# puzzlepaint/surfelmeshing

Hardware: AMD Instinct MI355X
Metric: RGB-D frames/s integrated @640x480, 5M live surfels; achieved HBM GB/s (higher is better)
Workload: dtype f32; 1 GPU; C2: synthetic room stream 640x480, raw depth + colour frames resident in HBM, full preprocessing + Integrate per frame, 4912850 live surfels (6250000 slots), steady-state re-traversal; max_surfel_count=6250000, streams=1, parallelism=1 independent stream per GPU

## Files before the change

### surfelmeshing_amd/csrc/smx_recon.hip

```cpp
#include <math.h>
#include <cmath>
#include <stdlib.h>
#include <string.h>

#include <algorithm>
#include <atomic>
#include <vector>

#include "smx_recon_state.hpp"
#include "smx_mesh.hpp"
#include <hip/hip_ext.h>

using namespace smx;

namespace {

struct FrameCtx {
  Mat34 L;
  Mat34 G;
  float fx, fy, cx, cy;
  Unproj up;
  float inv_depth_scaling;
  float sensor_noise_factor;
  float cos_normal_compat;
// ... 654 lines not shown
  SMX_STAMP(stamps, 2);
  if (lane == 0) {
    tb.count[tile * kCountStride] = 0;
    if (tile == 0) { *next_ovf_count = 0; seg_work_count[0] = 0; seg_work_count[1] = 0; }
    if (c.stats) {
      atomicAdd(&st->n_pairs, n_total);
      atomicMax(&st->max_tile_pairs, n_total);
      if (tile == 0) st->n_overflow_pairs = n_ovf;
    }
  }
#pragma unroll
  for (int q = 0; q < kPairCache; ++q) if (have[q]) assoc_stage(t, c, rec[q]);
  for_uncached_pairs(S, c, tb, tile, n_binned, overflowed, n_ovf, [&](const PairRec& r) { assoc_stage(t, c, r); });
  __syncthreads();
  SMX_STAMP(stamps, 3);
  uint32_t cand[kPairCache];
  float4 cp4[kPairCache], cn4[kPairCache];
#pragma unroll
  for (int q = 0; q < kPairCache; ++q) cand[q] = have[q] ? merge_candidate(t, c, rec[q]) : kInvalid;
#pragma unroll
  for (int q = 0; q < kPairCache; ++q) {
    const uint32_t g = cand[q] == kInvalid ? 0u : cand[q];
    cp4[q] = *S.group(kGroupP, g); cn4[q] = *S.group(kGroupN, g);
  }
#pragma unroll
  for (int q = 0; q < kPairCache; ++q) { keep(cp4[q]); keep(cn4[q]); }
#pragma unroll
  for (int q = 0; q < kPairCache; ++q) if (cand[q] != kInvalid) merge_decide(rec[q], cp4[q], cn4[q], merge_flag);
  for_uncached_pairs(S, c, tb, tile, n_binned, overflowed, n_ovf, [&](const PairRec& r) { merge_stage(t, S, c, r, merge_flag); });
  __syncthreads();
  SMX_STAMP(stamps, 4);
  if (in_image) {
    const size_t k = (size_t)y * c.W + x;
    sc.first_depth[k] = __int_as_float(t.zmin[lane]);
    sc.supporting[k] = t.sup[lane];
    sc.counts[k] = t.cnt[lane];
    sc.depth_sums[k] = (long long)t.sum[lane];
    sc.confl_key[k] = t.confl[lane];
  }
  SMX_STAMP(stamps, 5);
  ts_end(c.ts, kTsTilesEnd, blockIdx.x, gridDim.x);
}

__device__ __forceinline__ float depth_sum_avg(const Scratch& sc, size_t k) {
  return q_to_float(sc.depth_sums[k]) / (float)sc.counts[k];
}

__global__ void __launch_bounds__(kBlock)
k_blend_start(float ds, Img<uint16_t> depth, Scratch sc, BlendBufs b, int W, int H, unsigned long long* ts) {
  ts_end(ts, kTsBlendEnd, blockIdx.y * gridDim.x + blockIdx.x, gridDim.x * gridDim.y);
  const int x = blockIdx.x * 64 + (threadIdx.x & 63);
  const int y = blockIdx.y * 4 + (threadIdx.x >> 6);
  if (!(x >= 1 && y >= 1 && x < W - 1 && y < H - 1)) return;
  const size_t k = (size_t)y * W + x;
  const uint16_t own = depth(y, x);
  if (own == 0 || sc.supporting[k] == kInvalid) return;
  bool measurement_border = false, surfel_border = false;
  for (int wy = y - 1; wy <= y + 1; ++wy)
    for (int wx = x - 1; wx <= x + 1; ++wx) {
      if (depth(wy, wx) == 0) measurement_border = true;
      else if (sc.supporting[(size_t)wy * W + wx] == kInvalid) surfel_border = true;
    }
  if (surfel_border) {
    b.new_distance_map[k] = 1;
    const float avg = depth_sum_avg(sc, k);
    b.new_deltas[k] = avg - (float)own / ds;
  }
  if (measurement_border) {
    b.distance_map[k] = 1;
    const float avg = depth_sum_avg(sc, k);
    b.deltas[k] = avg - (float)own / ds;
// ... 264 lines not shown
#endif
    }
#ifdef SMX_STAMPS
    if (dbg) { dbg[0] = t_in; dbg[1] = wall_clock64(); dbg[2] = polls; }
#endif
  }
}

constexpr int kScanPxPerThread = 4;
constexpr int kScanPxPerBlock = kBlock * kScanPxPerThread;

struct NewFlagsArgs {
  Img<const uint16_t> depth; Img<uint16_t> depth_out; int copy_back;
  uint8_t* flags; uint32_t* local_rank; uint32_t* block_sums;
  unsigned long long* dbg;
};
__device__ __forceinline__ void new_flags_scan_body(const NewFlagsArgs& a, const Scratch& sc, int W, int H, DevState* st, uint32_t block) {
  const Img<const uint16_t>& depth = a.depth;
  const Img<uint16_t>& depth_out = a.depth_out;
  const int copy_back = a.copy_back;
  uint8_t* __restrict__ flags = a.flags;
  uint32_t* __restrict__ local_rank = a.local_rank;
  uint32_t* __restrict__ block_sums = a.block_sums;
  __shared__ uint32_t wave_tot[kBlock / 64];
  const int P = W * H;
  const int k0 = (block * kBlock + threadIdx.x) * kScanPxPerThread;
  uint32_t f[kScanPxPerThread];
  uint32_t mine = 0;
  uint32_t dv[kScanPxPerThread], sv[kScanPxPerThread], cv[kScanPxPerThread];
#pragma unroll
  for (int j = 0; j < kScanPxPerThread; ++j) {
    const int k = min(k0 + j, P - 1);
    const int y = k / W, x = k - y * W;
    dv[j] = depth(y, x); sv[j] = sc.supporting[k]; cv[j] = sc.confl_key[k];
  }
#pragma unroll
  for (int j = 0; j < kScanPxPerThread; ++j) { keep(dv[j]); keep(sv[j]); keep(cv[j]); }
#pragma unroll
  for (int j = 0; j < kScanPxPerThread; ++j) {
    const int k = k0 + j;
    bool fl = false;
    if (k < P) {
      const int y = k / W, x = k - y * W;
      const uint16_t d = (uint16_t)dv[j];
      if (copy_back) depth_out(y, x) = d;
      fl = x >= 1 && y >= 1 && x < W - 1 && y < H - 1 && d > 0 && sv[j] == kInvalid && cv[j] == kInvalid;
      flags[k] = fl ? 1 : 0;
    }
    f[j] = fl ? 1u : 0u;
    mine += f[j];
  }
  const uint32_t lane = threadIdx.x & 63, wave = threadIdx.x >> 6;
  uint32_t incl = mine;
#pragma unroll
  for (int off = 1; off < 64; off <<= 1) {
    const uint32_t t = __shfl_up(incl, off);
    if (lane >= (uint32_t)off) incl += t;
  }
  if (lane == 63) wave_tot[wave] = incl;
  __syncthreads();
  uint32_t wave_off = 0, total = 0;
#pragma unroll
  for (int w = 0; w < kBlock / 64; ++w) {
    if ((uint32_t)w < wave) wave_off += wave_tot[w];
    total += wave_tot[w];
  }
  uint32_t run = wave_off + incl - mine;
#pragma unroll
  for (int j = 0; j < kScanPxPerThread; ++j) {
    const int k = k0 + j;
    if (k < P) local_rank[k] = run;
    run += f[j];
  }
  if (threadIdx.x == 0) {
    block_sums[block] = total;
    if (block == 0) st->create_base_next = st->surfel_count;
  }
}

struct FrameIn {
  Img<const uint16_t> depth; Img<const float2> normals; Img<const float> radius; Img<const uchar3> color;
};

struct PixelIn {
  uint16_t depth; float first; uint32_t key; uint32_t count; float2 nxy; uchar3 col; float radius;
};
__device__ __forceinline__ PixelIn load_pixel(const FrameCtx& c, const Scratch& sc, const FrameIn& in, int x, int y) {
  const size_t k = (size_t)y * c.W + x;
  PixelIn p;
  p.depth = in.depth(y, x); p.first = sc.first_depth[k]; p.key = sc.confl_key[k]; p.count = sc.counts[k];
  p.nxy = in.normals(y, x); p.col = in.color(y, x); p.radius = in.radius(y, x);
  return p;
}

__device__ __forceinline__ void keep(const PixelIn& p) {
  keep((uint32_t)p.depth); keep(p.first); keep(p.key); keep(p.count); keep(p.nxy); keep(p.radius);
  keep((uint32_t)p.col.x | ((uint32_t)p.col.y << 8) | ((uint32_t)p.col.z << 16));
}

struct SurfelRegs {
  float4 P;
  float4 N;
  float4 C;
  bool dirty;
  bool replaced;
  Vec3 new_smooth;
};

__device__ __forceinline__ void integrate_or_conflict(SurfelRegs& R, const FrameCtx& c, const PixelIn& px,
                                                      bool integrate, int x, int y,
                                                      const Vec3& cam, uint32_t i, DevState* st) {
  if (!integrate) return;
  const float measurement_depth = c.inv_depth_scaling * (float)px.depth;
  if (measurement_depth <= 0) return;
  bool conflicting = false;
  const float first = px.first;
  if (first < (1 - c.sensor_noise_factor) * measurement_depth) {
    if (first == cam.z) {
      const uint32_t key = px.key;
      if (key != kInvalid && (key & 0x7FFFFFFFu) == i) conflicting = true;
    }
    integrate = false;
  }
// ... 104 lines not shown
    const float4 p4 = R.P, n4 = R.N;
    if (!is_active(__float_as_uint(p4.w), c.frame, c.window)) continue;
    Proj p;
    const Vec3 g = {p4.x, p4.y, p4.z};
    if (!project_pos(g, c, p)) continue;
    if (n4.w < 0) continue;
    int ox = p.px, oy = p.py;
    const bool second = quadrant(p, c, ox, oy);
    const PixelIn px0 = load_pixel(c, sc, in, p.px, p.py);
    const PixelIn px1 = load_pixel(c, sc, in, ox, oy);
    integrate_or_conflict(R, c, px0, true, p.px, p.py, p.l, i, st);
    integrate_or_conflict(R, c, px1, second, ox, oy, p.l, i, st);
    if (R.dirty) {
      L.hot_epoch[i >> L.hot_shift] = (uint8_t)L.epoch;
      if (L.dirty8) L.dirty8[i] = 1;
      out_store16(S.group(kGroupP, i), R.P); out_store16(S.group(kGroupN, i), R.N);
      out_store16(S.group(kGroupC, i), R.C);
      if (R.replaced) {
        *S.group(kGroupS, i) = make_float4(R.new_smooth.x, R.new_smooth.y, R.new_smooth.z, 0.0f);
        S.set_neighbors(i, make_uint4(kInvalid, kInvalid, kInvalid, kInvalid));
      }
    }
    L.flags8[i] = make_flags(__float_as_uint(R.P.w), __float_as_uint(R.C.z), c.frame, c.reg_window);
  }
#pragma unroll
  for (int off = 32; off > 0; off >>= 1) merged_here += __shfl_xor(merged_here, off);
  if ((threadIdx.x & 63) == 0 && merged_here) {
    atomicAdd(&st->merge_count, merged_here);
    if (c.stats) atomicAdd(&st->n_merged, merged_here);
  }
  ts_end(c.ts, kTsIntEnd, block, min(n_blocks, n_steps));
}

template <bool kUseList>
__device__ __forceinline__ void update_neighbors_body(const Surfels& S, const FrameCtx& c, const Scratch& sc, const FrameIn& in,
                                                      const Lists& L, const DevState* st, uint32_t block, uint32_t n_blocks) {
  const int kDX[4] = {-1, 1, 0, 0}, kDY[4] = {0, 0, -1, 1};
  const uint32_t n_scan = kUseList ? 0u : st->create_base_next;
  if (block == 0 && threadIdx.x < kSubLists) { L.rec_chunks.count[threadIdx.x * kCountStride] = 0; L.acc_chunks.count[threadIdx.x * kCountStride] = 0; }
  uint32_t ent, cntv;
  const uint32_t n_steps = vis_begin<kUseList>(L, n_scan, block, ent, cntv);
  for (uint32_t w = block; w < n_steps; w += n_blocks) {
    const uint32_t cur = ent;
    ent = (w + n_blocks < n_steps) ? vis_load<kUseList>(L, w + n_blocks) : 0u;
    uint32_t i;
    if (!vis_entry<kUseList>(cur, w, cntv, n_scan, threadIdx.x, i)) continue;
    const float4 p4 = *S.group(kGroupP, i), n4 = *S.group(kGroupN, i);
    const uint4 t4 = *reinterpret_cast<const uint4*>(S.group(kGroupT, i));
    if (!is_active(__float_as_uint(p4.w), c.frame, c.window)) continue;
    const Vec3 g = {p4.x, p4.y, p4.z};
    const Vec3 cam = mul(c.L, g);
    if (!(cam.z > 0)) continue;
    const float u = c.fx * (cam.x / cam.z) + c.cx, v = c.fy * (cam.y / cam.z) + c.cy;
    if (!(u >= 1.0f && v >= 1.0f && u < (float)(c.W - 1) && v < (float)(c.H - 1))) continue;
    const int x = (int)u, y = (int)v;
    const float measurement_depth = c.inv_depth_scaling * (float)in.depth(y, x);
    const float obs_r2 = in.radius(y, x);
    uint32_t cand[4];
#pragma unroll
    for (int d = 0; d < 4; ++d) cand[d] = sc.supporting[(size_t)(y + kDY[d]) * c.W + (x + kDX[d])];
    const float occlusion_depth = (1 + c.sensor_noise_factor) * measurement_depth;
    if (cam.z > occlusion_depth) continue;
    const float surfel_distance = sqrtf(cam.x * cam.x + cam.y * cam.y + cam.z * cam.z);
    const Vec3 gn = {n4.x, n4.y, n4.z};
    const Vec3 ln = rotate(c.L, gn);
    const float dot_angle = (1.0f / surfel_distance) * (cam.x * ln.x + cam.y * ln.y + cam.z * ln.z);
    if (dot_angle > 0) continue;
    const float r2 = n4.w;
    if (r2 < 0) continue;
    if (obs_r2 / r2 > 1.5f * 1.5f) continue;

    uint32_t ni[4] = {t4.x, t4.y, t4.z, t4.w};
    float4 np4[4], cp4[4], cn4[4];
#pragma unroll
    for (int q = 0; q < 4; ++q) np4[q] = *S.group(kGroupP, ni[q] == kInvalid ? i : ni[q]);
#pragma unroll
    for (int d = 0; d < 4; ++d) {
      const uint32_t gidx = (cand[d] == kInvalid) ? i : cand[d];
      cp4[d] = *S.group(kGroupP, gidx);
      cn4[d] = *S.group(kGroupN, gidx);
    }
    float nd2[4];
#pragma unroll
    for (int q = 0; q < 4; ++q) {
      if (ni[q] == kInvalid) nd2[q] = __builtin_inff();
      else {
        const float dx = g.x - np4[q].x, dy = g.y - np4[q].y, dz = g.z - np4[q].z;
        nd2[q] = dx * dx + dy * dy + dz * dz;
      }
    }
#pragma unroll
    for (int d = 0; d < 4; ++d) {
      const uint32_t nb = cand[d];
      if (nb == kInvalid || nb == i) continue;
      const float dx = cp4[d].x - g.x, dy = cp4[d].y - g.y, dz = cp4[d].z - g.z;
      const float d2 = dx * dx + dy * dy + dz * dz;
      if (d2 > c.rf2 * r2) continue;
      const float nd = gn.x * cn4[d].x + gn.y * cn4[d].y + gn.z * cn4[d].z;
      if (nd <= 0) continue;
      int best_n = -1; float best_d2 = -1;
#pragma unroll
      for (int q = 0; q < 4; ++q) {
        if (best_n == -2) continue;
        if (nb == ni[q]) { best_n = -2; }
        else if (nd2[q] > best_d2) { best_n = q; best_d2 = nd2[q]; }
      }
      if (best_n >= 0 && d2 < best_d2) {
#pragma unroll
        for (int q = 0; q < 4; ++q) if (q == best_n) { ni[q] = nb; nd2[q] = d2; }
      }
    }
    if (ni[0] != t4.x || ni[1] != t4.y || ni[2] != t4.z || ni[3] != t4.w) {
      S.set_neighbors(i, make_uint4(ni[0], ni[1], ni[2], ni[3]));
      L.hot_epoch[i >> L.hot_shift] = (uint8_t)L.epoch;
    }
  }
  ts_end(c.ts, kTsUpdEnd, block, min(n_blocks, n_steps));
}

struct CreateArgs {
  const uint8_t* flags; const uint32_t* ranks; const uint32_t* block_sums; uint32_t* block_offsets_out;
  int n_scan_blocks; uint32_t max_surfels; uint8_t* flags8; uint8_t* dirty8;
  uint32_t* next_vis_chunk_count;
  int n_pixels;
  uint8_t* hot_epoch; uint32_t epoch; int hot_shift;
};
__device__ __forceinline__ void new_create_body(const Surfels& S, const FrameCtx& c, const Scratch& sc, const FrameIn& in,
                                                const CreateArgs& a, DevState* st, uint32_t block, uint32_t n_blocks) {
  const uint8_t* __restrict__ flags = a.flags;
  const uint32_t* __restrict__ ranks = a.ranks;
  const uint32_t* __restrict__ block_sums = a.block_sums;
  uint32_t* __restrict__ block_offsets_out = a.block_offsets_out;
  const int n_scan_blocks = a.n_scan_blocks;
  const uint32_t max_surfels = a.max_surfels;
  uint8_t* __restrict__ flags8 = a.flags8;
  extern __shared__ uint32_t block_offsets[];
  __shared__ uint32_t wave_tot[kBlock / 64];
  static_assert(kScanPxPerBlock % kBlock == 0, "a creating workgroup's pixels lie inside one scan block");
  if (block != 0 && n_blocks * (uint32_t)kBlock >= (uint32_t)(c.W * c.H) &&
      block_sums[(block * (uint32_t)kBlock) / (uint32_t)kScanPxPerBlock] == 0) return;
  const int per = (n_scan_blocks + kBlock - 1) / kBlock;
  const uint32_t base = st->create_base_next;
  uint32_t mine = 0, total;
  if (per <= 8) {
    uint32_t v[8];
#pragma unroll
    for (int j = 0; j < 8; ++j) {
      const int bidx = threadIdx.x * per + j;
// ... 765 lines not shown
    __syncthreads();
    if (threadIdx.x == 0) carry += total;
    __syncthreads();
  }
  if (threadIdx.x == 0) *total_out = carry;
}
__global__ void __launch_bounds__(kBlock)
k_delta_gather(Surfels S, uint8_t* __restrict__ dirty8, const uint32_t* __restrict__ seg_offset, float* __restrict__ out,
               uint32_t total, const DevState* st) {
  __shared__ uint32_t wave_tot[kBlock / 64];
  const uint32_t N = st->surfel_count, i0 = blockIdx.x * kSeg + threadIdx.x * 4;
  uint32_t bits = 0;
  if (i0 < N) {
    const uchar4 d = *reinterpret_cast<const uchar4*>(&dirty8[i0]);
    bits = (d.x != 0 ? 1u : 0u) | ((i0 + 1 < N && d.y != 0) ? 2u : 0u) | ((i0 + 2 < N && d.z != 0) ? 4u : 0u) |
           ((i0 + 3 < N && d.w != 0) ? 8u : 0u);
    if (bits) *reinterpret_cast<uchar4*>(&dirty8[i0]) = make_uchar4(0, 0, 0, 0);
  }
  uint32_t seg_total;
  uint32_t off = seg_offset[blockIdx.x] + block_excl_scan((uint32_t)__popc(bits), wave_tot, seg_total);
  const int want[8] = {kSmoothX, kSmoothY, kSmoothZ, kRadiusSq, kNormalX, kNormalY, kNormalZ, kLastUpdateStamp};
#pragma unroll
  for (int j = 0; j < 4; ++j)
    if (bits & (1u << j)) {
      const uint32_t i = i0 + j;
      out[off] = __uint_as_float(i);
#pragma unroll
      for (int k = 0; k < 8; ++k) out[(size_t)(k + 1) * total + off] = S.f(want[k], i);
      ++off;
    }
}

__global__ void __launch_bounds__(kBlock)
k_decode_conflicting(const uint32_t* __restrict__ key, uint32_t* __restrict__ out, int P) {
  const int k = blockIdx.x * kBlock + threadIdx.x;
  if (k < P) out[k] = (key[k] == kInvalid) ? kInvalid : (key[k] & 0x7FFFFFFFu);
}

__global__ void __launch_bounds__(kBlock)
k_global_ranks(const uint32_t* __restrict__ local_rank, const uint32_t* __restrict__ block_offsets,
               uint32_t* __restrict__ out, int P) {
  const int k = blockIdx.x * kBlock + threadIdx.x;
  if (k < P) out[k] = block_offsets[k / kScanPxPerBlock] + local_rank[k];
}

}

enum : int {
  kSlotScanVisible = 0, kSlotAssocTiles, kSlotBlend, kSlotIntegrate,
  kSlotUpdateNeighbors, kSlotNeighborScan,
  kSlotRegAccumulate, kSlotRegStep,
  kSlotRegUpdate,
  kSlotCull,
  kSlotEmpty,
  kSlotCount
};
static const char* const kSlotNames[kSlotCount] = {
  "scan_visible", "assoc_tiles", "blend", "integrate+new_flags", "update_neighbors+create",
  "neighbor_scan", "reg_accumulate", "reg_step", "reg_update", "cull_segments", "empty_slot"};

struct SlotTimer {
  smx_recon r; hipStream_t st; int slot; bool kev, prof, by_launch;
  SlotTimer(smx_recon r_, hipStream_t st_, int slot_, bool launch_carries = false) : r(r_), st(st_), slot(slot_) {
    kev = (r->timing_enabled & 2) != 0;
    prof = (r->prof_slot == slot) && r->prof_ev && r->prof_n < r->prof_cap;
    by_launch = prof && launch_carries;
    if (kev) (void)hipEventRecord(r->kev[2 * slot], st);
    if (prof && !by_launch) (void)hipEventRecord(r->prof_ev[2 * r->prof_n], st);
  }
// ... 145 lines not shown
  SMX_TRY(r->mem.alloc(&r->fb.count, ((size_t)r->nsegB + 1) * kCountStride, true));
  r->L.vis_region = (uint32_t)(div_up(r->nseg, kSubLists) * kSeg);
  SMX_TRY(r->mem.alloc(&r->L.vis_list, (size_t)kSubLists * r->L.vis_region, true));
  SMX_TRY(r->mem.alloc(&r->L.recent_list, (size_t)r->nsegB * kSegB, false));
  SMX_TRY(r->mem.alloc(&r->L.vis_seg, (size_t)r->nseg, true));
  SMX_TRY(r->mem.alloc(&r->L.seg_box, (size_t)r->nseg * 8, true));
  SMX_TRY(r->mem.alloc(&r->L.seg_act, (size_t)r->nseg, true));
  SMX_TRY(r->mem.alloc(&r->L.seg_streak, (size_t)r->nseg, true));
  SMX_TRY(r->mem.alloc(&r->sw.surv_list, (size_t)r->nseg + 65536, true));
  SMX_TRY(r->mem.alloc(&r->sw.copy_list, (size_t)r->nseg + 65536, true));
  SMX_TRY(r->mem.alloc(&r->sw.count, 2, true));
  SMX_TRY(r->mem.alloc_host(&r->dir_host, 2, true));
  r->dir_host[0] = 0;
  r->dir_host[1] = 0;
  SMX_TRY(hip_rc(hipHostGetDevicePointer(reinterpret_cast<void**>(&r->dir_dev), r->dir_host, 0), "hipHostGetDevicePointer"));
  SMX_TRY(r->mem.alloc(&r->L.recent_seg, (size_t)r->nsegB, true));
  r->L.vis_chunks.stride = 0; r->L.vis_chunks.desc = nullptr;
  r->L.rec_chunks.stride = (uint32_t)(div_up(r->nsegB, kSubLists) + 8192);
  SMX_TRY(r->mem.alloc(&r->L.rec_chunks.desc, (size_t)kSubLists * r->L.rec_chunks.stride, true));
  SMX_TRY(r->mem.alloc(&r->L.rec_chunks.count, (size_t)kSubLists * kCountStride, true));
  static_assert(kSegAcc == kSegB && kAccCount < kCountStride, "pass B lists the edge kernel's segments by its own segment numbers");
  r->L.acc_chunks.stride = r->L.rec_chunks.stride;
  r->L.acc_chunks.count = r->L.rec_chunks.count + kAccCount;
  SMX_TRY(r->mem.alloc(&r->L.acc_chunks.desc, (size_t)kSubLists * r->L.acc_chunks.stride, true));
  SMX_TRY(r->mem.alloc(&r->flags_buf[0], (size_t)r->nsegB * kSegB, true));
  SMX_TRY(r->mem.alloc(&r->flags_buf[1], (size_t)r->nsegB * kSegB, true));
  r->L.flags8 = r->flags_buf[0];
  r->L.hot_shift = 10;
  while ((((size_t)r->nseg * kSeg) >> r->L.hot_shift) + 1 > (size_t)kMaxHotGroups) ++r->L.hot_shift;
  r->L.n_hot_groups = (uint32_t)((((size_t)r->nseg * kSeg) >> r->L.hot_shift) + 1);
  SMX_TRY(r->mem.alloc(&r->L.hot_epoch, (size_t)r->L.n_hot_groups + 64, true));
  SMX_TRY(r->mem.alloc(&r->L.seg_targets, (size_t)r->nsegB * kBlockB, true));
  r->L.epoch = 128;
  r->hot_filter_enabled = 1;
  r->fuse_edges = kFuseEdgesDefault;
  r->hot_holdoff = 3;
  SMX_TRY(r->mem.alloc(&r->merge_flag, r->S.pitch, true));
  SMX_TRY(r->mem.alloc(&r->gate_count, 32, true));
  r->gate_expected = 0;
  constexpr int kHandoverModeDefault = 1;
  r->handover_mode = kHandoverModeDefault;
  {
    const char* cc = getenv("ROCPROF_COUNTER_COLLECTION");
    if (cc && cc[0] && strcmp(cc, "0") != 0) r->handover_mode = 0;
  }
  SMX_TRY(r->mem.alloc(&r->L.act_list, (size_t)r->nsegB * kSegB, true));
  SMX_TRY(r->mem.alloc(&r->sc.supporting, P, true));
  SMX_TRY(r->mem.alloc(&r->sc.counts, P, true));
  SMX_TRY(r->mem.alloc(&r->sc.depth_sums, P, true));
  SMX_TRY(r->mem.alloc(&r->sc.confl_key, P, true));
  SMX_TRY(r->mem.alloc(&r->sc.first_depth, P, true));
  for (int k = 0; k < 2; ++k) {
    SMX_TRY(r->mem.alloc(&r->vis_count_set[k], (size_t)kSubLists * kCountStride, true));
    SMX_TRY(r->mem.alloc(&r->ovf_count_set[k], 1, true));
  }
  r->L.vis_chunks.count = r->vis_count_set[0];
  r->tb.tiles_x = div_up(width, kTileW);
  r->tb.n_tiles = (uint32_t)(r->tb.tiles_x * div_up(height, kTileH));
  r->tb.cap = r->bin_cap_full = kTileBinCap;
  SMX_TRY(r->mem.alloc(&r->tb.pairs, (size_t)r->tb.n_tiles * kTileBinCap, false));
  SMX_TRY(r->mem.alloc(&r->tb.count, (size_t)r->tb.n_tiles * kCountStride, true));
  SMX_TRY(r->mem.alloc(&r->tb.ovf, 2 * (size_t)r->S.pitch + 64, false));
  r->tb.ovf_count = r->ovf_count_set[0];
#ifdef SMX_STAMPS
  SMX_TRY(r->mem.alloc(&r->stamps, (size_t)3 * 16 * 8192, true));
#endif
  SMX_TRY(r->mem.alloc(&r->blended_depth, P, true));
  SMX_TRY(r->mem.alloc(&r->bb.distance_map, P, true));
  SMX_TRY(r->mem.alloc(&r->bb.new_distance_map, P, true));
  SMX_TRY(r->mem.alloc(&r->bb.deltas, P, true));
  SMX_TRY(r->mem.alloc(&r->bb.new_deltas, P, true));
  SMX_TRY(r->mem.alloc(&r->new_flags, P, true));
  SMX_TRY(r->mem.alloc(&r->new_ranks, P, true));
  SMX_TRY(r->mem.alloc(&r->tmp_u32, P, true));
  r->n_scan_blocks = div_up((long long)P, kScanPxPerBlock);
  SMX_TRY(r->mem.alloc(&r->block_sums, (size_t)r->n_scan_blocks, true));
  SMX_TRY(r->mem.alloc(&r->block_offsets, (size_t)r->n_scan_blocks, true));
  SMX_TRY(r->mem.alloc(&r->st, 1, true));
  SMX_TRY(r->mem.alloc(&r->ts_ring, (size_t)kTsRing * kTsWords, true));
  SMX_TRY(r->mem.alloc_host(&r->ts_host, (size_t)kTsRing * kTsWords, false));
  SMX_TRY(r->mem.alloc_host(&r->ts_mapped, (size_t)kTsRing * kTsWords, true));
  memset(const_cast<unsigned long long*>(r->ts_mapped), 0, sizeof(unsigned long long) * kTsRing * kTsWords);
  SMX_TRY(hip_rc(hipHostGetDevicePointer(reinterpret_cast<void**>(&r->ts_mapped_dev), const_cast<unsigned long long*>(r->ts_mapped), 0), "hipHostGetDevicePointer"));
  SMX_TRY(hip_rc(hipDeviceGetAttribute(&r->wall_khz, hipDeviceAttributeWallClockRate, device), "hipDeviceGetAttribute"));
// ... 90 lines not shown
  *avg_ms = r->prof_n ? (float)(sum / r->prof_n) : 0.0f;
  r->prof_slot = -1;
  return SMX_OK;
}

int smx_recon_set_stats_enabled(smx_recon r, int32_t enabled) {
  SMX_CHECK_ARG(r != nullptr);
  SMX_ON_DEVICE(r->device);
  r->stats_enabled = enabled ? 1 : 0;
  return SMX_OK;
}

int smx_recon_set_overlap(smx_recon r, int32_t enabled) {
  SMX_CHECK_ARG(r != nullptr && (enabled == 0 || enabled == 1));
  SMX_ON_DEVICE(r->device);
  if (r->reg_pending) { SMX_HIP(hipStreamSynchronize(r->reg_stream)); r->reg_pending = false; }
  r->overlap_enabled = enabled;
  return SMX_OK;
}

int smx_recon_set_handover_mode(smx_recon r, int32_t mode) {
  SMX_CHECK_ARG(r != nullptr && (mode == 0 || mode == 1));
  r->handover_mode = mode;
  return SMX_OK;
}

int smx_recon_get_handover_mode(smx_recon r, int32_t* mode) {
  SMX_CHECK_ARG(r != nullptr && mode != nullptr);
  *mode = r->handover_mode;
  return SMX_OK;
}

int smx_recon_set_scan_mode(smx_recon r, int32_t mode) {
  SMX_CHECK_ARG(r != nullptr && mode >= 0 && mode <= 1023);
  SMX_ON_DEVICE(r->device);
  r->grid_list = ((mode >> 8) & 1) ? 4 : r->grid_list_full;
  r->scan_mode = mode & 1;
  r->blend_multi_launch = (mode >> 1) & 1;
  r->hot_filter_enabled = ((mode >> 2) & 1) ? 0 : 1;
  r->tb.cap = ((mode >> 3) & 1) ? 16u : r->bin_cap_full;
  r->no_lds_tables = (mode >> 4) & 1;
  r->fb.cap = ((mode >> 5) & 1) ? 4u : kFarBinCap;
  r->fb.hash_mask = ((mode >> 6) & 1) ? 1u : (uint32_t)kFarHash - 1u;
  r->fuse_edges = ((mode >> 9) & 1) ? 1 : kFuseEdgesDefault;
  r->blend_other_tile = (mode >> 7) & 1;
  return SMX_OK;
}

int smx_recon_debug_set_skip(smx_recon r, int32_t mask) {
  SMX_CHECK_ARG(r != nullptr && mask >= 0 && mask <= 511);
  r->debug_skip = mask;
  return SMX_OK;
}

int smx_recon_integrate(smx_recon r, smx_stream s, uint32_t frame_index, float depth_scaling,
                        const smx_buffer_desc* depth, const smx_buffer_desc* normals,
                        const smx_buffer_desc* radius, const smx_buffer_desc* color,
                        const float global_T_local[12], const smx_integrate_params* p) {
  SMX_CHECK_ARG(r != nullptr);
  const hipEvent_t hook_consumed = r->hook_consumed, hook_chain = r->hook_chain, hook_ready = r->hook_ready;
  r->hook_consumed = nullptr; r->hook_chain = nullptr; r->hook_ready = nullptr;
  SMX_CHECK_ARG(depth && normals && radius && color && global_T_local && p);
  SMX_ON_DEVICE(r->device);
  SMX_CHECK_ARG(depth->width == r->W && depth->height == r->H && normals->width == r->W && normals->height == r->H);
  SMX_CHECK_ARG(radius->width == r->W && radius->height == r->H && color->width == r->W && color->height == r->H);
  SMX_CHECK_ARG(!p->do_blending || (p->measurement_blending_radius >= 2 && p->measurement_blending_radius <= 255));
  hipStream_t st = (hipStream_t)s;
  if (r->have_frame && (int32_t)(frame_index - r->last_frame) < 0) {
    SMX_CALL(join_regularizer(r, st));
    SMX_HIP(hipMemsetAsync(r->L.vis_seg, 0, (size_t)r->nseg * 4, st));
    SMX_HIP(hipMemsetAsync(r->L.seg_box, 0, (size_t)r->nseg * 8 * sizeof(float), st));
    r->hot_holdoff = 3;
  }
  r->have_frame = true; r->last_frame = frame_index;
  if (r->handover_mode == 1 && reinterpret_cast<volatile uint32_t*>(r->dir_host)[1] != 0u) r->handover_mode = 0;
  FrameCtx c;
  memcpy(c.G.m, global_T_local, sizeof(float) * 12);
  c.L = se3_inverse(global_T_local);
// ... 378 lines not shown
  d->frame_index = frame_index;
  d->surfel_count = n;
  d->count = total;
  if (total > d->capacity) {
    set_error("delta of %u slots does not fit the capacity %u", total, d->capacity);
    return SMX_ERR_INVALID_ARGUMENT;
  }
  if (total == 0) return SMX_OK;
  SMX_CHECK_ARG(d->surfel_index && d->x && d->y && d->z && d->radius_squared && d->normal_x && d->normal_y &&
                d->normal_z && d->last_update_stamp);
  SMX_CALL(acquire_staging(r, st, (size_t)9 * total));
  hipLaunchKernelGGL(k_delta_gather, dim3(r->nseg), dim3(kBlock), 0, st, r->S, r->L.dirty8, r->delta_seg.get(), r->staging.buf.get(), total,
                     r->st);
  SMX_LAUNCH_CHECK();
  void* dst[9] = {d->surfel_index, d->x, d->y, d->z, d->radius_squared, d->normal_x, d->normal_y, d->normal_z,
                  d->last_update_stamp};
  for (int k = 0; k < 9; ++k)
    SMX_HIP(hipMemcpyAsync(dst[k], r->staging.buf.get() + (size_t)k * total, (size_t)total * 4, hipMemcpyDeviceToHost, st));
  SMX_HIP(hipStreamSynchronize(st));
  return SMX_OK;
}

int smx_recon_debug_download_scratch(smx_recon r, smx_stream s, int32_t which, void* dst) {
  SMX_CHECK_ARG(r != nullptr && dst != nullptr);
  SMX_ON_DEVICE(r->device);
  SMX_CALL(join_regularizer(r, (hipStream_t)s));
  hipStream_t st = (hipStream_t)s;
  const size_t P = (size_t)r->W * r->H;
  const void* src = nullptr; size_t bytes = 0;
  switch (which) {
    case SMX_SCRATCH_SUPPORTING: src = r->sc.supporting; bytes = P * 4; break;
    case SMX_SCRATCH_SUPPORT_COUNTS: src = r->sc.counts; bytes = P * 4; break;
    case SMX_SCRATCH_DEPTH_SUMS: src = r->sc.depth_sums; bytes = P * 8; break;
    case SMX_SCRATCH_FIRST_DEPTH: src = r->sc.first_depth; bytes = P * 4; break;
    case SMX_SCRATCH_NEW_FLAGS: src = r->new_flags; bytes = P; break;
    case SMX_SCRATCH_CONFLICTING:
      hipLaunchKernelGGL(k_decode_conflicting, dim3(div_up((long long)P, kBlock)), dim3(kBlock), 0, st, r->sc.confl_key, r->tmp_u32, (int)P);
      src = r->tmp_u32; bytes = P * 4; break;
    case SMX_SCRATCH_NEW_INDICES:
      hipLaunchKernelGGL(k_global_ranks, dim3(div_up((long long)P, kBlock)), dim3(kBlock), 0, st, r->new_ranks, r->block_offsets, r->tmp_u32, (int)P);
      src = r->tmp_u32; bytes = P * 4; break;
    default: set_error("unknown scratch id %d", which); return SMX_ERR_INVALID_ARGUMENT;
  }
  SMX_HIP(hipMemcpyAsync(dst, src, bytes, hipMemcpyDeviceToHost, st));
  SMX_HIP(hipStreamSynchronize(st));
  return SMX_OK;
}

int smx_recon_debug_count_skipped_segments(smx_recon r, smx_stream s, uint32_t* out) {
  SMX_CHECK_ARG(r != nullptr && out != nullptr);
  SMX_ON_DEVICE(r->device);
  SMX_CALL(join_regularizer(r, (hipStream_t)s));
  std::vector<uint32_t> marks((size_t)r->nsegB);
  SMX_HIP(hipMemcpyAsync(marks.data(), r->L.recent_seg, marks.size() * 4, hipMemcpyDeviceToHost, (hipStream_t)s));
  SMX_HIP(hipStreamSynchronize((hipStream_t)s));
  uint32_t n = 0;
  for (uint32_t m : marks) n += m == kInvalid ? 1u : 0u;
  *out = n;
  return SMX_OK;
}

}
```

### surfelmeshing_amd/csrc/smx_recon_state.hpp

```cpp
#pragma once

#include "smx_common.hpp"
#include "smx_components.hpp"
#include "smx_decimate.hpp"
#include "smx_distance.hpp"
#include "smx_fill.hpp"
#include "smx_raycast.hpp"
#include "smx_render.hpp"
#include "smx_sample.hpp"
#include "smx_track.hpp"

namespace smx {

struct MeshWorkspace;

enum : int {
  kX = 0, kY = 1, kZ = 2, kSmoothX = 3, kSmoothY = 4, kSmoothZ = 5, kConfidence = 6, kRadiusSq = 7,
  kNormalX = 8, kNormalY = 9, kNormalZ = 10, kGradX = 11, kGradY = 12, kGradZ = 13,
  kCreationStamp = 17, kLastUpdateStamp = 18, kNeighbor0 = 19, kGradCount = 23, kColor = 24, kRows = 25
};

struct DevState {
  uint32_t surfel_count;
  uint32_t merge_count;
// ... 10 lines not shown
};

enum : int { kGroupP = 0, kGroupS, kGroupN, kGroupT, kGroupC, kGroupG, kGroups };
__host__ __device__ constexpr int row_group(int row) {
  return row <= 2 ? kGroupP : row <= 5 ? kGroupS : row == 6 ? kGroupC : row == 7 ? kGroupN : row <= 10 ? kGroupN
       : row <= 13 ? kGroupG : row <= 16 ? -1 : row == 17 ? kGroupC : row == 18 ? kGroupP : row <= 22 ? kGroupT
       : row == 24 ? kGroupC : -1;
}
__host__ __device__ constexpr int row_sub(int row) {
  return row <= 2 ? row : row <= 5 ? row - 3 : row == 6 ? 0 : row == 7 ? 3 : row <= 10 ? row - 8
       : row <= 13 ? row - 11 : row == 17 ? 1 : row == 18 ? 3 : row <= 22 ? row - 19 : row == 24 ? 2 : -1;
}
__host__ __device__ constexpr int group_start(int g) { return g; }
constexpr int kQuadsPerSlot = 6;
struct Surfels {
  float* base;
  size_t pitch;
  __host__ __device__ __forceinline__ size_t quad(int g, uint32_t i) const { return (size_t)group_start(g) * pitch + (size_t)i; }
  __device__ __forceinline__ float& f(int row, uint32_t i) const { return base[quad(row_group(row), i) * 4 + row_sub(row)]; }
  __device__ __forceinline__ uint32_t& u(int row, uint32_t i) const {
    return reinterpret_cast<uint32_t*>(base)[quad(row_group(row), i) * 4 + row_sub(row)];
  }
  __device__ __forceinline__ float4* group(int g, uint32_t i) const { return reinterpret_cast<float4*>(base) + quad(g, i); }
  __device__ __forceinline__ void set_neighbors(uint32_t i, const uint4& t) const { *reinterpret_cast<uint4*>(group(kGroupT, i)) = t; }
  __device__ __forceinline__ void set_neighbor(uint32_t i, int q, uint32_t v) const { u(kNeighbor0 + q, i) = v; }
  struct View { const float4* p; size_t stride; };
  View view(int g) const { return View{reinterpret_cast<const float4*>(base) + quad(g, 0), quad(g, 1) - quad(g, 0)}; }
};

struct Scratch {
  uint32_t* supporting;
  uint32_t* counts;
  long long* depth_sums;
  uint32_t* confl_key;
  float* first_depth;
};

constexpr int kBlock = 256;

inline unsigned blocks_for(uint32_t n) { return (unsigned)div_up(n, kBlock); }
inline bool finite_f(float v) { return v - v == 0.0f; }
inline bool ranges_overlap(const void* a, size_t a_bytes, const void* b, size_t b_bytes) {
  if (!a || !b || a_bytes == 0 || b_bytes == 0) return false;
  const uintptr_t a0 = (uintptr_t)a, b0 = (uintptr_t)b;
  return a0 < b0 + b_bytes && b0 < a0 + a_bytes;
}
inline unsigned long long word64(const uint32_t* h, int lo) { return ((unsigned long long)h[lo + 1] << 32) | h[lo]; }

constexpr int kSeg = 1024;
constexpr int kSegB = 1024;
constexpr int kBlockB = kSegB / 4;
constexpr uint32_t kCountStride = 32;
constexpr uint32_t kSubLists = 16;
struct Chunks { uint32_t* desc; uint32_t* count; uint32_t stride; };
struct Lists {
  Chunks vis_chunks, rec_chunks;
  Chunks acc_chunks;
  uint32_t* vis_list;
  uint32_t vis_region;
  float* seg_box;
  uint32_t* vis_seg;
  uint8_t* seg_streak;
  uint32_t* recent_list;
  uint32_t* recent_seg;
  uint32_t* act_list;
  uint8_t* flags8;
  uint8_t* dirty8;
  uint8_t* seg_act;
  uint32_t descending;
  uint8_t* hot_epoch;
  uint16_t* seg_targets;
  uint32_t n_hot_groups;
  uint32_t epoch;
  int hot_shift;
};

struct FarBins {
  uint4* rec;
  uint32_t* count;
  uint32_t cap;
  uint32_t hash_mask;
};

struct TileBins {
  uint2* pairs;
  uint32_t* count;
  uint4* ovf;
  uint32_t* ovf_count;
  uint32_t cap;
  int tiles_x;
  uint32_t n_tiles;
};

template <int kWaves = kBlock / 64>
__device__ __forceinline__ uint32_t block_excl_scan(uint32_t mine, uint32_t* wave_tot , uint32_t& total) {
  const uint32_t lane = threadIdx.x & 63, wave = threadIdx.x >> 6;
  uint32_t incl = mine;
#pragma unroll
  for (int off = 1; off < 64; off <<= 1) {
    const uint32_t t = __shfl_up(incl, off);
    if (lane >= (uint32_t)off) incl += t;
  }
// ... 200 lines not shown
```

Before: 6104 frames/s.

## Pack per-pixel association scratch into uint4 and range-guard neighbor relink gathers

Replaces the separate first_depth and confl_key scratch arrays with one uint4 assoc array (zmin, conflict key, count, supporting), so the new-flags scan and pixel loads each issue a single 16-byte load instead of several scalar loads. The neighbor-update relink logic moves into a helper that filters out duplicate and invalid candidates early and returns before any gathers when none remain. Candidate gathers use AMDGPU raw buffer loads with a bounded resource descriptor, so invalid slots read zero without per-lane index selects; a plain path is kept for very large pitches or when a mode bit selects it. The cost is redundant writes of support and count into both the packed array and the old arrays, and extra scratch bytes per pixel.

```diff
diff --git a/surfelmeshing_amd/csrc/smx_recon.hip b/surfelmeshing_amd/csrc/smx_recon.hip
--- a/surfelmeshing_amd/csrc/smx_recon.hip
+++ b/surfelmeshing_amd/csrc/smx_recon.hip
@@ -710,11 +710,11 @@
   SMX_STAMP(stamps, 4);
   if (in_image) {
     const size_t k = (size_t)y * c.W + x;
-    sc.first_depth[k] = __int_as_float(t.zmin[lane]);
-    sc.supporting[k] = t.sup[lane];
-    sc.counts[k] = t.cnt[lane];
+    const uint32_t sup = t.sup[lane], cnt = t.cnt[lane];
+    sc.assoc[k] = make_uint4((uint32_t)t.zmin[lane], t.confl[lane], cnt, sup);
+    sc.supporting[k] = sup;
+    sc.counts[k] = cnt;
     sc.depth_sums[k] = (long long)t.sum[lane];
-    sc.confl_key[k] = t.confl[lane];
   }
   SMX_STAMP(stamps, 5);
   ts_end(c.ts, kTsTilesEnd, blockIdx.x, gridDim.x);
@@ -1045,7 +1045,8 @@
   for (int j = 0; j < kScanPxPerThread; ++j) {
     const int k = min(k0 + j, P - 1);
     const int y = k / W, x = k - y * W;
-    dv[j] = depth(y, x); sv[j] = sc.supporting[k]; cv[j] = sc.confl_key[k];
+    const uint4 a4 = sc.assoc[k];
+    dv[j] = depth(y, x); sv[j] = a4.w; cv[j] = a4.y;
   }
 #pragma unroll
   for (int j = 0; j < kScanPxPerThread; ++j) { keep(dv[j]); keep(sv[j]); keep(cv[j]); }
@@ -1101,7 +1102,8 @@
 __device__ __forceinline__ PixelIn load_pixel(const FrameCtx& c, const Scratch& sc, const FrameIn& in, int x, int y) {
   const size_t k = (size_t)y * c.W + x;
   PixelIn p;
-  p.depth = in.depth(y, x); p.first = sc.first_depth[k]; p.key = sc.confl_key[k]; p.count = sc.counts[k];
+  const uint4 a4 = sc.assoc[k];
+  p.depth = in.depth(y, x); p.first = __uint_as_float(a4.x); p.key = a4.y; p.count = a4.z;
   p.nxy = in.normals(y, x); p.col = in.color(y, x); p.radius = in.radius(y, x);
   return p;
 }
@@ -1272,6 +1274,74 @@
   ts_end(c.ts, kTsIntEnd, block, min(n_blocks, n_steps));
 }
 
+constexpr size_t kRangedGatherMaxPitch = (size_t)1 << 28;
+template <bool kRanged>
+struct RecordGather {
+  typedef uint32_t u32x4 __attribute__((ext_vector_type(4)));
+  __amdgpu_buffer_rsrc_t rs;
+  const float4* base;
+  __device__ __forceinline__ RecordGather(const Surfels& S, int g) : base(S.group(g, 0)) {
+    if (kRanged) rs = __builtin_amdgcn_make_buffer_rsrc(const_cast<float4*>(base), 0, (int)((uint32_t)S.pitch * 16u), 0x00020000);
+  }
+  __device__ __forceinline__ float4 at(uint32_t slot, uint32_t self) const {
+    if (!kRanged) return base[slot == kInvalid ? self : slot];
+    const u32x4 v = __builtin_amdgcn_raw_buffer_load_b128(rs, (int)(slot * 16u), 0, 0);
+    return make_float4(__uint_as_float(v.x), __uint_as_float(v.y), __uint_as_float(v.z), __uint_as_float(v.w));
+  }
+};
+
+template <bool kRanged>
+__device__ __forceinline__ void relink(const Surfels& S, const FrameCtx& c, const Lists& L, uint32_t i, const Vec3& g, const Vec3& gn,
+                                       float r2, const uint4& t4, uint32_t (&cand)[4]) {
+  uint32_t ni[4] = {t4.x, t4.y, t4.z, t4.w};
+#pragma unroll
+  for (int d = 0; d < 4; ++d)
+    if (cand[d] == i || cand[d] == t4.x || cand[d] == t4.y || cand[d] == t4.z || cand[d] == t4.w) cand[d] = kInvalid;
+  if ((cand[0] & cand[1] & cand[2] & cand[3]) == kInvalid) return;
+  const RecordGather<kRanged> gather_p(S, kGroupP), gather_n(S, kGroupN);
+  float4 np4[4], cp4[4], cn4[4];
+#pragma unroll
+  for (int q = 0; q < 4; ++q) np4[q] = *S.group(kGroupP, ni[q] == kInvalid ? i : ni[q]);
+#pragma unroll
+  for (int d = 0; d < 4; ++d) { cp4[d] = gather_p.at(cand[d], i); cn4[d] = gather_n.at(cand[d], i); }
+#pragma unroll
+  for (int q = 0; q < 4; ++q) { keep(np4[q].x); keep(np4[q].y); keep(np4[q].z); }
+  float nd2[4];
+#pragma unroll
+  for (int q = 0; q < 4; ++q) {
+    if (ni[q] == kInvalid) nd2[q] = __builtin_inff();
+    else {
+      const float dx = g.x - np4[q].x, dy = g.y - np4[q].y, dz = g.z - np4[q].z;
+      nd2[q] = dx * dx + dy * dy + dz * dz;
+    }
+  }
+#pragma unroll
+  for (int d = 0; d < 4; ++d) {
+    const uint32_t nb = cand[d];
+    if (nb == kInvalid) continue;
+    const float dx = cp4[d].x - g.x, dy = cp4[d].y - g.y, dz = cp4[d].z - g.z;
+    const float d2 = dx * dx + dy * dy + dz * dz;
+    if (d2 > c.rf2 * r2) continue;
+    const float nd = gn.x * cn4[d].x + gn.y * cn4[d].y + gn.z * cn4[d].z;
+    if (nd <= 0) continue;
+    int best_n = -1; float best_d2 = -1;
+#pragma unroll
+    for (int q = 0; q < 4; ++q) {
+      if (best_n == -2) continue;
+      if (nb == ni[q]) { best_n = -2; }
+      else if (nd2[q] > best_d2) { best_n = q; best_d2 = nd2[q]; }
+    }
+    if (best_n >= 0 && d2 < best_d2) {
+#pragma unroll
+      for (int q = 0; q < 4; ++q) if (q == best_n) { ni[q] = nb; nd2[q] = d2; }
+    }
+  }
+  if (ni[0] != t4.x || ni[1] != t4.y || ni[2] != t4.z || ni[3] != t4.w) {
+    S.set_neighbors(i, make_uint4(ni[0], ni[1], ni[2], ni[3]));
+    L.hot_epoch[i >> L.hot_shift] = (uint8_t)L.epoch;
+  }
+}
+
 template <bool kUseList>
 __device__ __forceinline__ void update_neighbors_body(const Surfels& S, const FrameCtx& c, const Scratch& sc, const FrameIn& in,
                                                       const Lists& L, const DevState* st, uint32_t block, uint32_t n_blocks) {
@@ -1310,50 +1380,8 @@
     if (r2 < 0) continue;
     if (obs_r2 / r2 > 1.5f * 1.5f) continue;
 
-    uint32_t ni[4] = {t4.x, t4.y, t4.z, t4.w};
-    float4 np4[4], cp4[4], cn4[4];
-#pragma unroll
-    for (int q = 0; q < 4; ++q) np4[q] = *S.group(kGroupP, ni[q] == kInvalid ? i : ni[q]);
-#pragma unroll
-    for (int d = 0; d < 4; ++d) {
-      const uint32_t gidx = (cand[d] == kInvalid) ? i : cand[d];
-      cp4[d] = *S.group(kGroupP, gidx);
-      cn4[d] = *S.group(kGroupN, gidx);
-    }
-    float nd2[4];
-#pragma unroll
-    for (int q = 0; q < 4; ++q) {
-      if (ni[q] == kInvalid) nd2[q] = __builtin_inff();
-      else {
-        const float dx = g.x - np4[q].x, dy = g.y - np4[q].y, dz = g.z - np4[q].z;
-        nd2[q] = dx * dx + dy * dy + dz * dz;
-      }
-    }
-#pragma unroll
-    for (int d = 0; d < 4; ++d) {
-      const uint32_t nb = cand[d];
-      if (nb == kInvalid || nb == i) continue;
-      const float dx = cp4[d].x - g.x, dy = cp4[d].y - g.y, dz = cp4[d].z - g.z;
-      const float d2 = dx * dx + dy * dy + dz * dz;
-      if (d2 > c.rf2 * r2) continue;
-      const float nd = gn.x * cn4[d].x + gn.y * cn4[d].y + gn.z * cn4[d].z;
-      if (nd <= 0) continue;
-      int best_n = -1; float best_d2 = -1;
-#pragma unroll
-      for (int q = 0; q < 4; ++q) {
-        if (best_n == -2) continue;
-        if (nb == ni[q]) { best_n = -2; }
-        else if (nd2[q] > best_d2) { best_n = q; best_d2 = nd2[q]; }
-      }
-      if (best_n >= 0 && d2 < best_d2) {
-#pragma unroll
-        for (int q = 0; q < 4; ++q) if (q == best_n) { ni[q] = nb; nd2[q] = d2; }
-      }
-    }
-    if (ni[0] != t4.x || ni[1] != t4.y || ni[2] != t4.z || ni[3] != t4.w) {
-      S.set_neighbors(i, make_uint4(ni[0], ni[1], ni[2], ni[3]));
-      L.hot_epoch[i >> L.hot_shift] = (uint8_t)L.epoch;
-    }
+    if (L.plain_gathers) relink<false>(S, c, L, i, g, gn, r2, t4, cand);
+    else relink<true>(S, c, L, i, g, gn, r2, t4, cand);
   }
   ts_end(c.ts, kTsUpdEnd, block, min(n_blocks, n_steps));
 }
@@ -2185,9 +2213,11 @@
 }
 
 __global__ void __launch_bounds__(kBlock)
-k_decode_conflicting(const uint32_t* __restrict__ key, uint32_t* __restrict__ out, int P) {
+k_decode_assoc(const uint4* __restrict__ assoc, uint32_t* __restrict__ out, int P, int first_depth) {
   const int k = blockIdx.x * kBlock + threadIdx.x;
-  if (k < P) out[k] = (key[k] == kInvalid) ? kInvalid : (key[k] & 0x7FFFFFFFu);
+  if (k >= P) return;
+  const uint4 a = assoc[k];
+  out[k] = first_depth ? a.x : (a.y == kInvalid) ? kInvalid : (a.y & 0x7FFFFFFFu);
 }
 
 __global__ void __launch_bounds__(kBlock)
@@ -2399,6 +2429,7 @@
   SMX_TRY(r->mem.alloc(&r->L.hot_epoch, (size_t)r->L.n_hot_groups + 64, true));
   SMX_TRY(r->mem.alloc(&r->L.seg_targets, (size_t)r->nsegB * kBlockB, true));
   r->L.epoch = 128;
+  r->L.plain_gathers = r->S.pitch >= kRangedGatherMaxPitch ? 1u : 0u;
   r->hot_filter_enabled = 1;
   r->fuse_edges = kFuseEdgesDefault;
   r->hot_holdoff = 3;
@@ -2415,8 +2446,7 @@
   SMX_TRY(r->mem.alloc(&r->sc.supporting, P, true));
   SMX_TRY(r->mem.alloc(&r->sc.counts, P, true));
   SMX_TRY(r->mem.alloc(&r->sc.depth_sums, P, true));
-  SMX_TRY(r->mem.alloc(&r->sc.confl_key, P, true));
-  SMX_TRY(r->mem.alloc(&r->sc.first_depth, P, true));
+  SMX_TRY(r->mem.alloc(&r->sc.assoc, P, true));
   for (int k = 0; k < 2; ++k) {
     SMX_TRY(r->mem.alloc(&r->vis_count_set[k], (size_t)kSubLists * kCountStride, true));
     SMX_TRY(r->mem.alloc(&r->ovf_count_set[k], 1, true));
@@ -2573,7 +2603,7 @@
 }
 
 int smx_recon_set_scan_mode(smx_recon r, int32_t mode) {
-  SMX_CHECK_ARG(r != nullptr && mode >= 0 && mode <= 1023);
+  SMX_CHECK_ARG(r != nullptr && mode >= 0 && mode <= 2047);
   SMX_ON_DEVICE(r->device);
   r->grid_list = ((mode >> 8) & 1) ? 4 : r->grid_list_full;
   r->scan_mode = mode & 1;
@@ -2585,6 +2615,7 @@
   r->fb.hash_mask = ((mode >> 6) & 1) ? 1u : (uint32_t)kFarHash - 1u;
   r->fuse_edges = ((mode >> 9) & 1) ? 1 : kFuseEdgesDefault;
   r->blend_other_tile = (mode >> 7) & 1;
+  r->L.plain_gathers = (((mode >> 10) & 1) || r->S.pitch >= kRangedGatherMaxPitch) ? 1u : 0u;
   return SMX_OK;
 }
 
@@ -3029,10 +3060,11 @@
     case SMX_SCRATCH_SUPPORTING: src = r->sc.supporting; bytes = P * 4; break;
     case SMX_SCRATCH_SUPPORT_COUNTS: src = r->sc.counts; bytes = P * 4; break;
     case SMX_SCRATCH_DEPTH_SUMS: src = r->sc.depth_sums; bytes = P * 8; break;
-    case SMX_SCRATCH_FIRST_DEPTH: src = r->sc.first_depth; bytes = P * 4; break;
     case SMX_SCRATCH_NEW_FLAGS: src = r->new_flags; bytes = P; break;
+    case SMX_SCRATCH_FIRST_DEPTH:
     case SMX_SCRATCH_CONFLICTING:
-      hipLaunchKernelGGL(k_decode_conflicting, dim3(div_up((long long)P, kBlock)), dim3(kBlock), 0, st, r->sc.confl_key, r->tmp_u32, (int)P);
+      hipLaunchKernelGGL(k_decode_assoc, dim3(div_up((long long)P, kBlock)), dim3(kBlock), 0, st, r->sc.assoc, r->tmp_u32, (int)P,
+                         which == SMX_SCRATCH_FIRST_DEPTH ? 1 : 0);
       src = r->tmp_u32; bytes = P * 4; break;
     case SMX_SCRATCH_NEW_INDICES:
       hipLaunchKernelGGL(k_global_ranks, dim3(div_up((long long)P, kBlock)), dim3(kBlock), 0, st, r->new_ranks, r->block_offsets, r->tmp_u32, (int)P);
diff --git a/surfelmeshing_amd/csrc/smx_recon_state.hpp b/surfelmeshing_amd/csrc/smx_recon_state.hpp
--- a/surfelmeshing_amd/csrc/smx_recon_state.hpp
+++ b/surfelmeshing_amd/csrc/smx_recon_state.hpp
@@ -66,8 +66,7 @@
   uint32_t* supporting;
   uint32_t* counts;
   long long* depth_sums;
-  uint32_t* confl_key;
-  float* first_depth;
+  uint4* assoc;
 };
 
 constexpr int kBlock = 256;
@@ -102,6 +101,7 @@
   uint8_t* dirty8;
   uint8_t* seg_act;
   uint32_t descending;
+  uint32_t plain_gathers;
   uint8_t* hot_epoch;
   uint16_t* seg_targets;
   uint32_t n_hot_groups;
```

Result: faster. 6200 frames/s (median of 6 runs) (+1.6%).
